# ManuelZ/image-search-engine

Hardware: AMD Instinct MI355X
Metric: queries/sec, exact brute-force L2 kNN (recall@10 vs exact CPU), 1Mx512 fp32 index, k=10 (higher is better)
Workload: dtype f32; 1 GPU; 1000000x512 fp32 uniform[0,1) index (default_rng 1234), L2, k=10, nq=16 queries per step, index resident in HBM, steps issued round-robin on 16 HIP streams; 400 untimed steps ahead of the warm-up bring the GPU out of its idle power state; n=1000000, d=512, k=10, nq=16

## Files before the change

image-search-engine_amd/csrc/ise_exact.hpp:

```cpp
#pragma once
#include "ise_common.hpp"
#include "ise_select.hpp"

template <int R>
__device__ __forceinline__ void exact_l2_rows(const float* const (&rows)[R], const float* qs, int dp, int lane,
                                              float (&out)[R]) {
    float s[R];
#pragma unroll
    for (int r = 0; r < R; r++) s[r] = 0.f;
    for (int j = lane * 4; j < dp; j += 256) {
        const f32x4 x = *reinterpret_cast<const f32x4*>(qs + j);
        f32x4 y[R];
#pragma unroll
        for (int r = 0; r < R; r++) y[r] = *reinterpret_cast<const f32x4*>(rows[r] + j);
#pragma unroll
        for (int r = 0; r < R; r++) {
            const f32x4 t = y[r] - x;
            s[r] = fmaf(t[0], t[0], s[r]);
            s[r] = fmaf(t[1], t[1], s[r]);
            s[r] = fmaf(t[2], t[2], s[r]);
            s[r] = fmaf(t[3], t[3], s[r]);
        }
    }
#pragma unroll
    for (int r = 0; r < R; r++) out[r] = wave_sum_f32(s[r]);
}

struct ExactParams {
    const float* xb;
    const float* q;
    long long n;
    int d, dp, nq;
    int k;
    int kc;
    uint32_t id_base;
    float* D;
    long long* I;
    u64* keys_out;
    u64* fl_state;
    int* fl_list;
    uint32_t seq;
    unsigned long long* stats;
    int force_fail;
    const float* tau_bound;
};

__device__ __forceinline__ void fallback_list_push(const ExactParams& p, int q) {
    u64 old = __hip_atomic_load(p.fl_state, __ATOMIC_RELAXED, __HIP_MEMORY_SCOPE_AGENT);
    for (;;) {
        const u64 want = ((uint32_t)(old >> 32) == p.seq) ? old + 1 : (((u64)p.seq << 32) | 1ull);
        if (__hip_atomic_compare_exchange_strong(p.fl_state, &old, want, __ATOMIC_RELAXED, __ATOMIC_RELAXED,
                                                 __HIP_MEMORY_SCOPE_AGENT)) {
            p.fl_list[(uint32_t)want - 1] = q;
            return;
        }
    }
}

__device__ __forceinline__ void emit_exact(const ExactParams& p, size_t o, u64 key) {
    if (p.keys_out) p.keys_out[o] = key;
    if (p.D) {
        const bool pad = key == KEY_PAD;
        p.D[o] = pad ? FLT_MAX : unord_f32((uint32_t)(key >> 32));
        p.I[o] = pad ? -1ll : (long long)(uint32_t)key;
    }
}

__device__ __forceinline__ void block_sort_u64(u64* a, int n2, int tid, int nthreads) {
    for (int size = 2; size <= n2; size <<= 1)
        for (int stride = size >> 1; stride > 0; stride >>= 1) {
            __syncthreads();
            for (int i = tid; i < (n2 >> 1); i += nthreads) {
                const int lo = 2 * i - (i & (stride - 1)), hi = lo + stride;
                const bool up = (lo & size) == 0;
                const u64 x = a[lo], y = a[hi];
                if ((x > y) == up) {
                    a[lo] = y;
                    a[hi] = x;
                }
            }
        }
    __syncthreads();
}

__host__ __device__ constexpr int rerank_pow2(int kc) {
    int n2 = 1;
    while (n2 < kc) n2 <<= 1;
    return n2;
}
__host__ __device__ constexpr size_t rerank_lds_bytes(int dp, int kc) {
    return (size_t)dp * 4 + (size_t)kc * 8 + (size_t)rerank_pow2(kc) * 8;
}

template <int NT>
__device__ __forceinline__ void rerank_stage_query(const ExactParams& p, int q, unsigned char* smem) {
    float* qs = reinterpret_cast<float*>(smem);
    const float* src = p.q + (size_t)q * p.d;
    for (int j = threadIdx.x; j < p.dp; j += NT) qs[j] = j < p.d ? src[j] : 0.f;
}

template <int NT>
__device__ __forceinline__ void rerank_block(const ExactParams& p, int q, unsigned char* smem,
                                             const u64* keys_in_global) {
    constexpr int NW = NT / 64;
    float* qs = reinterpret_cast<float*>(smem);
    u64* kin = reinterpret_cast<u64*>(qs + p.dp);
    u64* kex = kin + p.kc;
    const int tid = threadIdx.x, lane = tid & 63, w = __builtin_amdgcn_readfirstlane(tid >> 6);
    const int n2 = rerank_pow2(p.kc);
    DBG_STAMP(p.stats ? p.stats + 8 : nullptr, 3);
    if (keys_in_global)
        for (int c = tid; c < p.kc; c += NT) kin[c] = keys_in_global[(size_t)q * p.kc + c];
    __syncthreads();
    int count = 0;
    for (int c0 = 0; c0 < p.kc; c0 += 64) {
        const bool real = (c0 + lane) < p.kc && kin[c0 + lane] != KEY_PAD;
        count += __popcll(__ballot(real));
    }
    DBG_STAMP(p.stats ? p.stats + 8 : nullptr, 4);
    constexpr int R = NW >= 8 ? 2 : 4;
    for (int c0 = w * R; c0 < n2; c0 += NW * R) {
        if (c0 >= count) {
            if (lane < R && c0 + lane < n2) kex[c0 + lane] = KEY_PAD;
            continue;
        }
        const float* rows[R];
        u64 kc_[R];
#pragma unroll
        for (int r = 0; r < R; r++) {
            const int c = c0 + r;
            kc_[r] = c < count ? kin[c] : KEY_PAD;
            const long long row = kc_[r] != KEY_PAD ? (long long)((uint32_t)kc_[r] - p.id_base) : 0ll;
            rows[r] = p.xb + (size_t)row * p.dp;
        }
        float dd[R];
        exact_l2_rows<R>(rows, qs, p.dp, lane, dd);
        if (lane == 0) {
#pragma unroll
            for (int r = 0; r < R; r++)
                if (c0 + r < n2)
                    kex[c0 + r] = (kc_[r] != KEY_PAD && dd[r] < FLT_MAX) ? (((u64)ord_f32(dd[r]) << 32) | (uint32_t)kc_[r])
                                                                       : KEY_PAD;
        }
    }
    DBG_STAMP(p.stats ? p.stats + 8 : nullptr, 5);
    if (n2 <= 64) {
        __syncthreads();
        if (w == 0) {
            const u64 mine = lane < n2 ? kex[lane] : KEY_PAD;
            int rk = 0;
            for (int j = 0; j < n2; j++) rk += readlane_u64(mine, j) < mine ? 1 : 0;
            const u64 padm = __ballot(mine == KEY_PAD) & ((lane < 63 ? (1ull << (lane + 1)) : 0ull) - 1ull);
            if (mine == KEY_PAD) rk += __popcll(padm) - 1;
            wave_lds_fence();
            if (lane < n2) kex[rk] = mine;
        }
        __syncthreads();
    } else {
        block_sort_u64(kex, n2, tid, NT);
    }
    DBG_STAMP(p.stats ? p.stats + 8 : nullptr, 6);
    bool ok = true;
    if (count == p.kc && p.n > p.kc) {
        const float lo_last = unord_f32((uint32_t)(kin[p.kc - 1] >> 32));
        const float d_k = unord_f32((uint32_t)(kex[p.k - 1] >> 32));
        ok = lo_last > d_k;
    }
    if (p.tau_bound) {
        if (count >= p.k) ok = ok && p.tau_bound[q] >= unord_f32((uint32_t)(kex[p.k - 1] >> 32));
        else ok = ok && (long long)count >= p.n;
    }
    if (p.force_fail) ok = false;
    for (int r = tid; r < p.k; r += NT) emit_exact(p, (size_t)q * p.k + r, r < count ? kex[r] : KEY_PAD);
    DBG_STAMP(p.stats ? p.stats + 8 : nullptr, 7);
    if (tid == 0) {
        if (p.stats) atomicAdd(&p.stats[0], 1ull);
        if (!ok) {
            if (p.stats) atomicAdd(&p.stats[1], 1ull);
            fallback_list_push(p, q);
        }
    }
}

static __global__ __launch_bounds__(256) void rerank_kernel(const ExactParams p, const u64* keys_in) {
    extern __shared__ __align__(16) unsigned char smem_rr[];
    rerank_stage_query<256>(p, (int)blockIdx.x, smem_rr);
    rerank_block<256>(p, (int)blockIdx.x, smem_rr, keys_in);
}
```

image-search-engine_amd/csrc/ise_merge.hpp:

```cpp
#pragma once
#include <climits>
#include <type_traits>

#include "ise_common.hpp"
#include "ise_exact.hpp"

#define MERGE_THREADS 512
#define MERGE_LISTS_MAX 1024
struct MergeParams {
    const u64* lists;
    long long stride_list;
    long long stride_qtile;
    int qt;
    int n_lists, nq, k, metric;
    int stride_query;
    float* D;
    long long* I;
    u64* keys_out;
    const u64* fl_state;
    const int* fl_list;
    uint32_t seq;
    int out_by_pos;
    unsigned long long* dbg;
    const unsigned int* gate;
};

__device__ __forceinline__ void emit_result(const MergeParams& p, size_t o, u64 key) {
    if (p.keys_out) p.keys_out[o] = key;
    if (p.D) {
        const bool pad = key == KEY_PAD;
        const float sc = unord_f32((uint32_t)(key >> 32));
        const bool l2 = p.metric == ISE_METRIC_L2;
        p.D[o] = pad ? (l2 ? FLT_MAX : -FLT_MAX) : (l2 ? sc : -sc);
        p.I[o] = pad ? -1ll : (long long)(uint32_t)key;
    }
}

template <int NT, int LPT>
struct ListHeads {
    const u64* lst[LPT];
    int pos[LPT];
    u64 cur[LPT], nxt[LPT];
    __device__ __forceinline__ void load(const MergeParams& p, const u64* base) {
#pragma unroll
        for (int e = 0; e < LPT; e++) {
            constexpr int NW = NT / 64;
            const int l = ((int)threadIdx.x & 63) * NW + ((int)threadIdx.x >> 6) + e * NT;
            const bool live = l < p.n_lists;
            lst[e] = base + (size_t)(live ? l : 0) * p.stride_list;
            pos[e] = 0;
            cur[e] = live ? lst[e][0] : KEY_PAD;
            nxt[e] = (live && p.k > 1) ? lst[e][1] : KEY_PAD;
        }
    }
    __device__ __forceinline__ u64 best() const {
        u64 m = cur[0];
#pragma unroll
        for (int e = 1; e < LPT; e++) m = min_u64(m, cur[e]);
        return m;
    }
    __device__ __forceinline__ bool advance(u64 m, int k) {
        bool mine = false;
#pragma unroll
        for (int e = 0; e < LPT; e++)
            if (cur[e] == m) {
                mine = true;
                pos[e]++;
                cur[e] = nxt[e];
                nxt[e] = pos[e] + 1 < k ? lst[e][pos[e] + 1] : KEY_PAD;
            }
        return mine;
    }
};

template <int NT, int LPT, typename Emit>
__device__ __forceinline__ void merge_rounds(const MergeParams& p, const u64* base, u64 (*wmin)[NT / 64], Emit emit) {
    const int tid = threadIdx.x, lane = tid & 63, w = __builtin_amdgcn_readfirstlane(tid >> 6);
    const int k = p.k;
    ListHeads<NT, LPT> h;
    h.load(p, base);
    for (int r = 0; r < k; r++) {
        u64 m = wave_min_u64(h.best());
        if (lane == 0) wmin[r & 1][w] = m;
        __syncthreads();
#pragma unroll
        for (int i = 0; i < NT / 64; i++) m = min_u64(m, wmin[r & 1][i]);
        if (m == KEY_PAD) {
            if (tid == 0) emit(r, KEY_PAD);
        } else if (h.advance(m, k)) {
            emit(r, m);
        }
    }
}

#define MERGE_FAST_K 40
#define MERGE_PRE 8
struct MergeFastScratch {
    u64 wl[MERGE_THREADS / 64][MERGE_FAST_K];
    int rank[64];
    int need_full;
};
__device__ __forceinline__ void merge_waves(const MergeParams& p, const u64* base, MergeFastScratch& s, u64* out) {
    constexpr int NW = MERGE_THREADS / 64, LPT = MERGE_LISTS_MAX / MERGE_THREADS;
    const int tid = threadIdx.x, lane = tid & 63, w = __builtin_amdgcn_readfirstlane(tid >> 6);
    const int k = p.k;
    ListHeads<MERGE_THREADS, LPT> h;
    h.load(p, base);
    DBG_STAMP(p.dbg, 1);
    u64 mine = KEY_PAD;
    const int pre = k < MERGE_PRE ? k : MERGE_PRE;
    for (int r = 0; r < pre; r++) {
        const u64 m = wave_min_u64(h.best());
        if (lane == r) mine = m;
        if (m != KEY_PAD) (void)h.advance(m, k);
    }
    if (lane < MERGE_PRE) s.wl[w][lane] = mine;
    if (tid < 64) s.rank[tid] = 0;
    if (tid == 0) s.need_full = 0;
    DBG_STAMP(p.dbg, 2);
    __syncthreads();
    const u64 mykey = s.wl[lane >> 3][lane & 7];
    {
        int part = 0;
#pragma unroll
        for (int j = 0; j < 8; j++) part += readlane_u64(mykey, 8 * w + j) < mykey ? 1 : 0;
        if (part) atomicAdd(&s.rank[lane], part);
    }
    __syncthreads();
    if (w == 0) {
        const bool real = mykey != KEY_PAD;
        const int rk = s.rank[lane];
        const int nreal = __popcll(__ballot(real));
        const int nw = nreal < k ? nreal : k;
        if (real && rk < k) out[rk] = mykey;
        if (lane >= nw && lane < k) out[lane] = KEY_PAD;
        const u64 hit = __ballot(real && rk == k - 1);
        const u64 T = hit ? readlane_u64(mykey, __ffsll((long long)hit) - 1) : KEY_PAD;
        const u64 last = pre == MERGE_PRE ? s.wl[lane & 7][MERGE_PRE - 1] : KEY_PAD;
        const bool undone = lane < NW && pre < k && last < T;
        if (__ballot(undone) != 0ull && lane == 0) s.need_full = 1;
    }
    __syncthreads();
    if (s.need_full) {
        for (int r = pre; r < k; r++) {
            const u64 m = wave_min_u64(h.best());
            if (lane == r) mine = m;
            if (m != KEY_PAD) (void)h.advance(m, k);
        }
        __syncthreads();
        if (lane < MERGE_FAST_K) s.wl[w][lane] = mine;
        __syncthreads();
        if (w == 0) {
            constexpr int KPLM = (NW * MERGE_FAST_K + 63) / 64;
            static_assert(NW * MERGE_FAST_K % 64 == 0, "the waves' lists fill whole registers");
            u64 kk[KPLM];
#pragma unroll
            for (int e = 0; e < KPLM; e++) kk[e] = (&s.wl[0][0])[lane + 64 * e];
            u64 kth_unused;
            const int nw = wave_select<KPLM>(kk, NW * MERGE_FAST_K, k, out, &kth_unused);
            if (lane >= nw && lane < k) out[lane] = KEY_PAD;
        }
        __syncthreads();
    }
}

template <bool RERANK>
__global__ __launch_bounds__(MERGE_THREADS) void merge_kernel(const MergeParams p, const ExactParams xp) {
    constexpr int LPT = MERGE_LISTS_MAX / MERGE_THREADS;
    __shared__ u64 wmin[2][MERGE_THREADS / 64];
    __shared__ MergeFastScratch fast;
    __shared__ u64 res[MERGE_FAST_K];
    extern __shared__ __align__(16) unsigned char smem_mr[];
    if (p.gate && *p.gate == 0u) return;
    int q = blockIdx.x, lq = blockIdx.x;
    if (p.fl_state) {
        const u64 st = __hip_atomic_load(p.fl_state, __ATOMIC_RELAXED, __HIP_MEMORY_SCOPE_AGENT);
        if ((uint32_t)(st >> 32) != p.seq || lq >= (int)(uint32_t)st) return;
        q = p.out_by_pos ? lq : p.fl_list[lq];
    }
    const int k = p.k;
    const u64* base = p.lists + (size_t)(lq / p.qt) * p.stride_qtile + (size_t)(lq % p.qt) * k;
    if (RERANK) {
        u64* kin = reinterpret_cast<u64*>(smem_mr + (size_t)xp.dp * 4);
        DBG_STAMP(xp.stats ? xp.stats + 8 : nullptr, 0);
        rerank_stage_query<MERGE_THREADS>(xp, q, smem_mr);
        if (k <= MERGE_FAST_K) merge_waves(p, base, fast, kin);
        else merge_rounds<MERGE_THREADS, LPT>(p, base, wmin, [&](int r, u64 key) { kin[r] = key; });
        rerank_block<MERGE_THREADS>(xp, q, smem_mr, nullptr);
    } else if (k <= MERGE_FAST_K) {
        merge_waves(p, base, fast, res);
        if ((int)threadIdx.x < k) emit_result(p, (size_t)q * k + threadIdx.x, res[threadIdx.x]);
    } else {
        merge_rounds<MERGE_THREADS, LPT>(p, base, wmin, [&](int r, u64 key) { emit_result(p, (size_t)q * k + r, key); });
    }
}

template <class T>
struct PassOut {
    T* D;
    long long* I;
    u64* lo;
    int k, off, ip;
    __device__ __forceinline__ void store(size_t at, u64 key, bool pad) const {
        if constexpr (std::is_same_v<T, float>) {
            const float sc = unord_f32((uint32_t)(key >> 32));
            D[at] = pad ? (ip ? -FLT_MAX : FLT_MAX) : (ip ? -sc : sc);
        } else {
            D[at] = pad ? INT_MAX : (int)((uint32_t)(key >> 32) - 1u);
        }
        I[at] = pad ? -1ll : (long long)(uint32_t)key;
    }
};

template <class T>
__global__ __launch_bounds__(MERGE_THREADS) void pass_merge_kernel(const MergeParams p, const PassOut<T> o) {
    __shared__ MergeFastScratch fast;
    __shared__ u64 res[MERGE_FAST_K];
    const int lq = blockIdx.x;
    merge_waves(p, p.lists + (size_t)lq * p.stride_query, fast, res);
    const int t = threadIdx.x;
    if (t < p.k) {
        const u64 key = res[t];
        const bool pad = key == KEY_PAD;
        o.store((size_t)lq * o.k + o.off + t, key, pad);
        if (t == p.k - 1) o.lo[lq] = pad ? KEY_PAD : key + 1;
    }
}

template <class T>
__global__ __launch_bounds__(256) void knn_fill_kernel(const PassOut<T> o, long long cnt) {
    const long long i = (long long)blockIdx.x * blockDim.x + threadIdx.x;
    if (i < cnt) o.store((size_t)i, KEY_PAD, true);
}

static __global__ __launch_bounds__(256) void merge_small_kernel(const MergeParams p) {
    const int lane = threadIdx.x & 63;
    const int q = blockIdx.x * 4 + (threadIdx.x >> 6);
    if (q >= p.nq) return;
    const int k = p.k;
    const u64* lst = p.lists + (size_t)(q / p.qt) * p.stride_qtile + (size_t)(q % p.qt) * k +
                     (size_t)(lane < p.n_lists ? lane : 0) * p.stride_list;
    const bool live = lane < p.n_lists;
    int pos = 0;
    u64 cur = live ? lst[0] : KEY_PAD;
    u64 nxt = (live && k > 1) ? lst[1] : KEY_PAD;
    for (int r = 0; r < k; r++) {
        const u64 m = wave_min_u64(cur);
        const size_t o = (size_t)q * k + r;
        if (m == KEY_PAD) {
            if (lane == 0) emit_result(p, o, KEY_PAD);
        } else if (cur == m) {
            emit_result(p, o, m);
            pos++;
            cur = nxt;
            nxt = pos + 1 < k ? lst[pos + 1] : KEY_PAD;
        }
    }
}
```

Before: 179,500 queries/s.

## Software-pipeline rerank row loads and window merge list heads with query staging

The exact rerank loop now streams candidate rows through a two-deep register ring. It interleaves candidates across waves, using readlane to pull keys from a per-lane key register, so global loads for the next step are in flight while the current step's FMAs run. The merge's list-head structure now fetches a four-entry window per list, using 16-byte vector loads when alignment allows, instead of one head at a time. Staging the query into LDS is overlapped with those initial list loads. This targets latency-bound global loads in a small-batch merge+rerank kernel, at the cost of more registers and more complex indexing.

```diff
diff --git a/image-search-engine_amd/csrc/ise_exact.hpp b/image-search-engine_amd/csrc/ise_exact.hpp
--- a/image-search-engine_amd/csrc/ise_exact.hpp
+++ b/image-search-engine_amd/csrc/ise_exact.hpp
@@ -99,6 +99,18 @@
     for (int j = threadIdx.x; j < p.dp; j += NT) qs[j] = j < p.d ? src[j] : 0.f;
 }
 
+#define RERANK_ROWS 4
+
+struct RerankCursor {
+    int g = 0, j = 0;
+    __device__ __forceinline__ void next(int nj) {
+        if (++j == nj) {
+            j = 0;
+            g++;
+        }
+    }
+};
+
 template <int NT>
 __device__ __forceinline__ void rerank_block(const ExactParams& p, int q, unsigned char* smem,
                                              const u64* keys_in_global) {
@@ -112,35 +124,85 @@
     if (keys_in_global)
         for (int c = tid; c < p.kc; c += NT) kin[c] = keys_in_global[(size_t)q * p.kc + c];
     __syncthreads();
+    const int nj = (p.dp + 255) >> 8;
+    int kb = 0;
+    auto lane_key = [&]() -> u64 { return (w + NW * (kb + lane)) < p.kc ? kin[w + NW * (kb + lane)] : KEY_PAD; };
+    u64 lanekey = lane_key();
+    f32x4 ring[2][RERANK_ROWS];
+    RerankCursor ld;
+    auto load_step = [&](f32x4(&y)[RERANK_ROWS]) {
+        const int j = (ld.j << 8) + lane * 4;
+        if (ld.g * RERANK_ROWS - kb >= 64) {
+            kb += 64;
+            lanekey = lane_key();
+        }
+#pragma unroll
+        for (int r = 0; r < RERANK_ROWS; r++) {
+            const u64 key = readlane_u64(lanekey, ld.g * RERANK_ROWS + r - kb);
+            if (key != KEY_PAD && j < p.dp)
+                y[r] = *reinterpret_cast<const f32x4*>(p.xb + (size_t)((uint32_t)key - p.id_base) * p.dp + j);
+        }
+        ld.next(nj);
+    };
+#pragma unroll
+    for (int h = 0; h < 2; h++) {
+#pragma unroll
+        for (int r = 0; r < RERANK_ROWS; r++) ring[h][r] = (f32x4){0.f, 0.f, 0.f, 0.f};
+        load_step(ring[h]);
+    }
     int count = 0;
     for (int c0 = 0; c0 < p.kc; c0 += 64) {
         const bool real = (c0 + lane) < p.kc && kin[c0 + lane] != KEY_PAD;
         count += __popcll(__ballot(real));
     }
     DBG_STAMP(p.stats ? p.stats + 8 : nullptr, 4);
-    constexpr int R = NW >= 8 ? 2 : 4;
-    for (int c0 = w * R; c0 < n2; c0 += NW * R) {
-        if (c0 >= count) {
-            if (lane < R && c0 + lane < n2) kex[c0 + lane] = KEY_PAD;
-            continue;
-        }
-        const float* rows[R];
-        u64 kc_[R];
-#pragma unroll
-        for (int r = 0; r < R; r++) {
-            const int c = c0 + r;
-            kc_[r] = c < count ? kin[c] : KEY_PAD;
-            const long long row = kc_[r] != KEY_PAD ? (long long)((uint32_t)kc_[r] - p.id_base) : 0ll;
-            rows[r] = p.xb + (size_t)row * p.dp;
-        }
-        float dd[R];
-        exact_l2_rows<R>(rows, qs, p.dp, lane, dd);
-        if (lane == 0) {
-#pragma unroll
-            for (int r = 0; r < R; r++)
-                if (c0 + r < n2)
-                    kex[c0 + r] = (kc_[r] != KEY_PAD && dd[r] < FLT_MAX) ? (((u64)ord_f32(dd[r]) << 32) | (uint32_t)kc_[r])
-                                                                       : KEY_PAD;
+    for (int c = count + tid; c < n2; c += NT) kex[c] = KEY_PAD;
+    {
+        const int rows_w = count > w ? (count - w + NW - 1) / NW : 0;
+        const int T = (rows_w + RERANK_ROWS - 1) / RERANK_ROWS * nj;
+        RerankCursor use;
+        float s[RERANK_ROWS];
+#pragma unroll
+        for (int r = 0; r < RERANK_ROWS; r++) s[r] = 0.f;
+        auto use_step = [&](f32x4(&slot)[RERANK_ROWS]) {
+            f32x4 y[RERANK_ROWS];
+#pragma unroll
+            for (int r = 0; r < RERANK_ROWS; r++) y[r] = slot[r];
+            load_step(slot);
+            const int j = (use.j << 8) + lane * 4;
+            if (j < p.dp) {
+                const f32x4 x = *reinterpret_cast<const f32x4*>(qs + j);
+#pragma unroll
+                for (int r = 0; r < RERANK_ROWS; r++) {
+                    const f32x4 t = y[r] - x;
+                    s[r] = fmaf(t[0], t[0], s[r]);
+                    s[r] = fmaf(t[1], t[1], s[r]);
+                    s[r] = fmaf(t[2], t[2], s[r]);
+                    s[r] = fmaf(t[3], t[3], s[r]);
+                }
+            }
+            if (use.j == nj - 1) {
+#pragma unroll
+                for (int o = 32; o > 0; o >>= 1) {
+                    float t[RERANK_ROWS];
+#pragma unroll
+                    for (int r = 0; r < RERANK_ROWS; r++) t[r] = __shfl_xor(s[r], o);
+#pragma unroll
+                    for (int r = 0; r < RERANK_ROWS; r++) s[r] += t[r];
+                }
+#pragma unroll
+                for (int r = 0; r < RERANK_ROWS; r++) {
+                    const int i = use.g * RERANK_ROWS + r;
+                    if (lane == 0 && i < rows_w)
+                        kex[w + NW * i] = s[r] < FLT_MAX ? (((u64)ord_f32(s[r]) << 32) | (uint32_t)kin[w + NW * i]) : KEY_PAD;
+                    s[r] = 0.f;
+                }
+            }
+            use.next(nj);
+        };
+        for (int t = 0; t < T; t += 2) {
+            use_step(ring[0]);
+            if (t + 1 < T) use_step(ring[1]);
         }
     }
     DBG_STAMP(p.stats ? p.stats + 8 : nullptr, 5);
diff --git a/image-search-engine_amd/csrc/ise_merge.hpp b/image-search-engine_amd/csrc/ise_merge.hpp
--- a/image-search-engine_amd/csrc/ise_merge.hpp
+++ b/image-search-engine_amd/csrc/ise_merge.hpp
@@ -36,8 +36,91 @@
     }
 }
 
+#define MERGE_WIN 4
+typedef u64 u64x2 __attribute__((ext_vector_type(2)));
 template <int NT, int LPT>
 struct ListHeads {
+    const u64* lst[LPT];
+    int used[LPT];
+    u64 win[LPT][MERGE_WIN];
+    bool vec;
+    __device__ __forceinline__ void request(int e, int at, int k) {
+        if (vec) {
+#pragma unroll
+            for (int i = 0; i < MERGE_WIN; i += 2) {
+                const int j = at + i;
+                const u64x2 v = *reinterpret_cast<const u64x2*>(lst[e] + (j < k ? j : k - 2));
+                win[e][i] = v[0];
+                win[e][i + 1] = v[1];
+            }
+        } else {
+#pragma unroll
+            for (int i = 0; i < MERGE_WIN; i++) {
+                const int j = at + i;
+                win[e][i] = lst[e][j < k ? j : k - 1];
+            }
+        }
+    }
+    __device__ __forceinline__ void settle(int e) {
+#pragma unroll
+        for (int i = 0; i < MERGE_WIN; i++) asm volatile("" : "+v"(win[e][i]));
+    }
+    __device__ __forceinline__ void mask(int e, int at, int k, bool live) {
+#pragma unroll
+        for (int i = 0; i < MERGE_WIN; i++)
+            if (!live || at + i >= k) win[e][i] = KEY_PAD;
+    }
+    template <typename Between>
+    __device__ __forceinline__ void load(const MergeParams& p, const u64* base, Between between) {
+        vec = ((p.k | (int)(p.stride_list & 1)) & 1) == 0 && (reinterpret_cast<uintptr_t>(base) & 15) == 0;
+        bool live[LPT];
+#pragma unroll
+        for (int e = 0; e < LPT; e++) {
+            constexpr int NW = NT / 64;
+            const int l = ((int)threadIdx.x & 63) * NW + ((int)threadIdx.x >> 6) + e * NT;
+            live[e] = l < p.n_lists;
+            lst[e] = base + (size_t)(live[e] ? l : 0) * p.stride_list;
+            used[e] = 0;
+        }
+#pragma unroll
+        for (int e = 0; e < LPT; e++) request(e, 0, p.k);
+        between();
+#pragma unroll
+        for (int e = 0; e < LPT; e++) settle(e);
+#pragma unroll
+        for (int e = 0; e < LPT; e++) mask(e, 0, p.k, live[e]);
+    }
+    __device__ __forceinline__ void load(const MergeParams& p, const u64* base) {
+        load(p, base, [] {});
+    }
+    __device__ __forceinline__ u64 best() const {
+        u64 m = win[0][0];
+#pragma unroll
+        for (int e = 1; e < LPT; e++) m = min_u64(m, win[e][0]);
+        return m;
+    }
+    __device__ __forceinline__ bool advance(u64 m, int k) {
+        bool mine = false;
+#pragma unroll
+        for (int e = 0; e < LPT; e++)
+            if (win[e][0] == m) {
+                mine = true;
+                used[e]++;
+#pragma unroll
+                for (int i = 0; i + 1 < MERGE_WIN; i++) win[e][i] = win[e][i + 1];
+                win[e][MERGE_WIN - 1] = KEY_PAD;
+                if ((used[e] & (MERGE_WIN - 1)) == 0 && used[e] < k) {
+                    request(e, used[e], k);
+                    settle(e);
+                    mask(e, used[e], k, true);
+                }
+            }
+        return mine;
+    }
+};
+
+template <int NT, int LPT>
+struct ListHeadsRounds {
     const u64* lst[LPT];
     int pos[LPT];
     u64 cur[LPT], nxt[LPT];
@@ -77,7 +160,7 @@
 __device__ __forceinline__ void merge_rounds(const MergeParams& p, const u64* base, u64 (*wmin)[NT / 64], Emit emit) {
     const int tid = threadIdx.x, lane = tid & 63, w = __builtin_amdgcn_readfirstlane(tid >> 6);
     const int k = p.k;
-    ListHeads<NT, LPT> h;
+    ListHeadsRounds<NT, LPT> h;
     h.load(p, base);
     for (int r = 0; r < k; r++) {
         u64 m = wave_min_u64(h.best());
@@ -100,12 +183,14 @@
     int rank[64];
     int need_full;
 };
-__device__ __forceinline__ void merge_waves(const MergeParams& p, const u64* base, MergeFastScratch& s, u64* out) {
+template <typename Between>
+__device__ __forceinline__ void merge_waves(const MergeParams& p, const u64* base, MergeFastScratch& s, u64* out,
+                                            Between between) {
     constexpr int NW = MERGE_THREADS / 64, LPT = MERGE_LISTS_MAX / MERGE_THREADS;
     const int tid = threadIdx.x, lane = tid & 63, w = __builtin_amdgcn_readfirstlane(tid >> 6);
     const int k = p.k;
     ListHeads<MERGE_THREADS, LPT> h;
-    h.load(p, base);
+    h.load(p, base, between);
     DBG_STAMP(p.dbg, 1);
     u64 mine = KEY_PAD;
     const int pre = k < MERGE_PRE ? k : MERGE_PRE;
@@ -164,6 +249,10 @@
     }
 }
 
+__device__ __forceinline__ void merge_waves(const MergeParams& p, const u64* base, MergeFastScratch& s, u64* out) {
+    merge_waves(p, base, s, out, [] {});
+}
+
 template <bool RERANK>
 __global__ __launch_bounds__(MERGE_THREADS) void merge_kernel(const MergeParams p, const ExactParams xp) {
     constexpr int LPT = MERGE_LISTS_MAX / MERGE_THREADS;
@@ -183,9 +272,12 @@
     if (RERANK) {
         u64* kin = reinterpret_cast<u64*>(smem_mr + (size_t)xp.dp * 4);
         DBG_STAMP(xp.stats ? xp.stats + 8 : nullptr, 0);
-        rerank_stage_query<MERGE_THREADS>(xp, q, smem_mr);
-        if (k <= MERGE_FAST_K) merge_waves(p, base, fast, kin);
-        else merge_rounds<MERGE_THREADS, LPT>(p, base, wmin, [&](int r, u64 key) { kin[r] = key; });
+        if (k <= MERGE_FAST_K) {
+            merge_waves(p, base, fast, kin, [&] { rerank_stage_query<MERGE_THREADS>(xp, q, smem_mr); });
+        } else {
+            rerank_stage_query<MERGE_THREADS>(xp, q, smem_mr);
+            merge_rounds<MERGE_THREADS, LPT>(p, base, wmin, [&](int r, u64 key) { kin[r] = key; });
+        }
         rerank_block<MERGE_THREADS>(xp, q, smem_mr, nullptr);
     } else if (k <= MERGE_FAST_K) {
         merge_waves(p, base, fast, res);
```

Measured after the change: 184,300 queries/s, median of 6. +2.7%, better.
